# mochell/PiCLES

Hardware: AMD Instinct MI355X
Metric: particle_steps_per_sec (higher is better)
Workload: dtype f64

## Files before the change

### picles_amd/csrc/k_step.inc

```
#ifndef K_STEP_NAME
#define K_STEP_NAME k_step
#define K_STEP_WROW false
#include "k_step.inc"
#undef K_STEP_NAME
#undef K_STEP_WROW
#define K_STEP_NAME k_step_waverow
#define K_STEP_WROW true
#include "k_step.inc"
#undef K_STEP_NAME
#undef K_STEP_WROW
#else
template <bool FAST, bool TSIT, bool STATIC, bool METRIC, bool AUTO>
__global__ void __launch_bounds__(256, (FAST && !AUTO) ? 4 : (FAST ? 3 : 2)) K_STEP_NAME(KParams P, GridP G, Arrays A, double t_prev, double DT_prev,
                                                double t_start, double DT, int r0, int n0, int r1, int n1)
{
    constexpr bool WROW = K_STEP_WROW;
    static_assert(!WROW || (FAST && !METRIC), "k_step_waverow: specialised physics, Cartesian");
#ifdef PICLES_PHASE_CLOCK
    const unsigned long long pc0_ = __builtin_readcyclecounter();
    unsigned long long pc1_ = pc0_, pc2_ = pc0_, pc3_ = pc0_;
#endif
#ifdef PICLES_WAVE_LOG
    const unsigned long long wl0_ = __builtin_amdgcn_s_memrealtime();
    unsigned long long wl1_ = 0;
#endif
    dp_device_init(TSIT ? 1 : 0);
    order_sign_init();
    const long long ord_counts = order_counts(A);
    const int ord_entry = order_entry(A);
    const int mr_early = pull_reach_early(A);
    pm_device_init();
    long long t = 0;
    const unsigned int lblock = ordered_block(A, ord_counts, ord_entry);
    WaveRow wr = {0, 0, 0};
    const unsigned int lane = threadIdx.x & 63u;
    bool active;
    if constexpr (WROW) { active = rows_index_waverow(G, r0, n0, lblock, wr); t = wr.t0 + lane; }
    else active = rows_index(G, r0, n0, r1, n1, t, lblock);
    StepStats S = {{0u, 0u, 0u, 0}, 0u, 0u, 0u, 0u, 0u, 0u, 0};
    int rtile = -1, ccode = -1;
    if (active) {
        int i, jl;
        if constexpr (WROW) { i = wr.i0 + (int)lane; jl = wr.jl; }
        else { i = (int)(t % G.Nx); jl = (int)(t / G.Nx); }
        double s0 = 0.0, s1 = 0.0, s2 = 0.0;
        if constexpr (WROW) rmap_clear_ahead_waverow(A, wr, lane);
        else rmap_clear_ahead(A, t);
        const Arrays Av = WROW ? arrays_at(A, wr.t0) : A;
        const long long tx = WROW ? (long long)lane : t;
        constexpr bool PREFETCH = AUTO;
        unsigned char pf_pre = 0;
        Wind w_pre = {0.0, 0.0, 0.0, 0.0, 0.0, 0.0};
        double qold_pre = 0.0, uP_pre = 0.0, vP_pre = 0.0;
        int asw_pre = 0;
        if constexpr (PREFETCH) {
            pf_pre = Av.pflags[tx];
            w_pre = load_wind(P, Av, tx);
            if constexpr (WROW) w_pre.xi = (unsigned int)t;
            qold_pre = Av.qold[tx];
            asw_pre = Av.asw[tx];
            if (!STATIC) { uP_pre = Av.uP[tx]; vP_pre = Av.vP[tx]; }
        }
        if constexpr (WROW) {
            int cls;
            const int Rl = pull_reach_local_waverow(G, A, wr, lane, pull_reach(G, A, jl, mr_early), cls);
            pull_waverow(G, A, wr, lane, Rl, cls, s0, s1, s2);
        }
        else pull_any(G, A, i, jl, pull_reach_local(G, A, i, jl, pull_reach(G, A, jl, mr_early)), s0, s1, s2);
#ifdef PICLES_PHASE_CLOCK
        __asm__ volatile("" : "+v"(s0), "+v"(s1), "+v"(s2));
        pc1_ = __builtin_readcyclecounter();
#endif
#ifdef PICLES_WAVE_LOG
        __asm__ volatile("" : "+v"(s0), "+v"(s1), "+v"(s2));
        wl1_ = __builtin_amdgcn_s_memrealtime();
#endif
        unsigned char pf = PREFETCH ? pf_pre : Av.pflags[tx];
        __shared__ int stash_[WROW ? 1 : 5][256];
        if (pf & PF_STEPPED) {
            Wind w = PREFETCH ? w_pre : load_wind(P, Av, tx);
            if constexpr (WROW) w.xi = (unsigned int)t;
            Vec5 z = {0.0, 0.0, 0.0, 0.0, 0.0};
            double qold = PREFETCH ? qold_pre : Av.qold[tx], dtn = -1.0;
            int br = remesh_regs_lazy(P, pf, s0, s1, s2, DT_prev, z, STATIC ? &Av.u0[tx] : (PREFETCH ? &uP_pre : &Av.uP[tx]),
                                      STATIC ? &Av.v0[tx] : (PREFETCH ? &vP_pre : &Av.vP[tx]));
            int on = (br <= 1);
            int asw = AUTO ? (PREFETCH ? asw_pre : Av.asw[tx]) : 0;
            if (br == 1) { qold = PI_LNQOLDINIT; asw = ASW_FRESH; S.reseeds = 1; }
            unsigned int rs = S.reseeds;
            S.reseeds = 0;
            const int tid_ = threadIdx.x;
            if constexpr (WROW) stash_[0][tid_] = (int)pf | ((int)rs << 8);
            else {
                stash_[0][tid_] = (int)(unsigned int)((unsigned long long)t & 0xffffffffull); stash_[1][tid_] = (int)((unsigned long long)t >> 32);
                stash_[2][tid_] = i; stash_[3][tid_] = jl; stash_[4][tid_] = (int)pf | ((int)rs << 8);
            }
            int status;
            if (METRIC) status = advance_core<FAST, STATIC, true, TSIT, AUTO>(P, w, z, on, qold, dtn, t_start, DT, S, Av.m11[tx], Av.m22[tx], Av.pc[tx], &asw);
            else status = advance_core<FAST, STATIC, false, TSIT, AUTO>(P, w, z, on, qold, dtn, t_start, DT, S, 0.0, 0.0, 0.0, &asw);
#ifdef PICLES_PHASE_CLOCK
            __asm__ volatile("" : "+v"(z.lne));
            pc2_ = __builtin_readcyclecounter();
#endif
            KStepArgsPtr K = kargs_reload();
            const KParams Pb = K->P;
            const GridP Gb = K->G;
            const Arrays Ab = K->A;
            __asm__ volatile("" ::: "memory");
            const int tid2_ = threadIdx.x;
            WaveRow wrb = {0, 0, 0};
            long long tb;
            int ib = 0, jlb = 0, pr_;
            if constexpr (WROW) {
                wrb = waverow_of(Gb, K->r0, lblock);
                tb = wrb.t0 + (threadIdx.x & 63u);
                pr_ = stash_[0][tid2_];
            } else {
                tb = (long long)(((unsigned long long)(unsigned int)stash_[1][tid2_] << 32) | (unsigned int)stash_[0][tid2_]);
                ib = stash_[2][tid2_]; jlb = stash_[3][tid2_]; pr_ = stash_[4][tid2_];
            }
            const unsigned char pfb = (unsigned char)(pr_ & 0xff);
            const Arrays Abv = WROW ? arrays_at(Ab, wrb.t0) : Ab;
            const long long tbx = WROW ? (long long)(threadIdx.x & 63u) : tb;
            status = advance_guards(Pb, [&]() { Wind wg = load_wind(Pb, Abv, tbx); if constexpr (WROW) wg.xi = (unsigned int)tb; return wg; },
                                    z, dtn, K->t_start, K->DT, status, S);
            if (AUTO) Abv.asw[tbx] = asw;
            S.reseeds += (unsigned int)(pr_ >> 8);
            Abv.qold[tbx] = qold;
            Abv.status[tbx] = status;
            if constexpr (WROW) write_record_at(Gb, rec_row_out(Ab, Gb, wrb.jl + Gb.R) + wrb.i0, threadIdx.x & 63u, pfb, on, z, S, &ccode);
            else write_record(Gb, Ab, ib, jlb, pfb, on, z, S);
            rtile = WROW ? (int)(wrb.t0 >> 6) : (int)(tb >> 6);
        }
    }
    {
        KStepArgsPtr K = kargs_reload();
        const Arrays Ab = K->A;
        flush_stats<WROW>(Ab, S, rtile, ccode);
        if (Ab.ord && order_wanted(Ab)) order_file(Ab, lblock, __ballot(S.adv != 0 || S.reseeds != 0) != 0);
#ifdef PICLES_WAVE_LOG
        if ((threadIdx.x & 63) == 0) {
            unsigned int hw_, xcc_;
            __asm__ volatile("s_getreg_b32 %0, hwreg(HW_REG_HW_ID)" : "=s"(hw_));
            __asm__ volatile("s_getreg_b32 %0, hwreg(HW_REG_XCC_ID)" : "=s"(xcc_));
            unsigned long long *wl_ = (unsigned long long *)Ab.movie + 4ull * ((unsigned long long)lblock * 4ull + (threadIdx.x >> 6));
            wl_[0] = wl0_; wl_[1] = wl1_; wl_[2] = __builtin_amdgcn_s_memrealtime();
            wl_[3] = (unsigned long long)hw_ | ((unsigned long long)xcc_ << 32) | ((unsigned long long)blockIdx.x << 40);
        }
#endif
#ifdef PICLES_PHASE_CLOCK
        pc3_ = __builtin_readcyclecounter();
        if ((threadIdx.x & 63) == 0) {
            DevCounters *c = Ab.cnt + ((blockIdx.x * 4u + (threadIdx.x >> 6)) & (NSLOTS - 1));
            if (pc1_ == pc0_) pc1_ = pc3_;
            if (pc2_ < pc1_) pc2_ = pc1_;
            atomicAdd(&c->pad_[0], pc1_ - pc0_); atomicAdd(&c->pad_[1], pc2_ - pc1_); atomicAdd(&c->pad_[2], pc3_ - pc2_); atomicAdd(&c->pad_[3], 1ull);
        }
#endif
    }
}
#endif
```

### picles_amd/csrc/kernels.h

```cpp
#ifndef PICLES_KERNELS_H
#define PICLES_KERNELS_H

#include <hip/hip_runtime.h>
#include <cstdint>
#include <type_traits>

#include "../../include/picles_hip.h"
#include "physics.h"

struct GridP {
    int Nx, Ny;
    int periodic_x, periodic_y;
    int tripolar;
    int j_begin, ny_loc;
    int R;
    int Rp;
    int single_slab;
    int ngroups;
};

#define NSLOTS 1024
struct DevCounters {
    unsigned long long rhs, acc, rej, reseeds, clamps, maxit, adv, overflow;
    unsigned long long nonfinite, wslots, pad_[4];
// ... 575 lines not shown
                int jw = jj; if (jw < 0) jw += G.Ny; else if (jw >= G.Ny) jw -= G.Ny;
                row = jw + RO;
            } else {
                row = jl + dj + RO;
            }
            if (!rowok) continue;
#pragma unroll 1
            for (int si = 0; si < W; si++) {
                int qi = si + shx; if (qi >= W) qi -= W;
                int di = qi - R;
                int ii = i + di;
                if (ii < 0 || ii >= Nx) {
                    if (!G.periodic_x) continue;
                    ii += (ii < 0) ? Nx : -Nx;
                }
                pull_candidate(rec, (unsigned int)row * rowlen + (unsigned int)ii, pl, di, dj, grp, true, s0, s1, s2);
            }
        }
    }
}

__device__ __forceinline__ int floor_mod(int a, int b) { int r = a % b; return (r < 0) ? r + b : r; }

__device__ __forceinline__ void pull_node_tripolar(const GridP &G, const Arrays &A, int i, int jl, int R,
                                                   double &s0, double &s1, double &s2)
{
    const int RO = G.R, Nx = G.Nx, Ny = G.Ny, j = jl + G.j_begin, W = 2 * R + 1;
    const double *__restrict__ rec = A.rec;
    const unsigned int pl = (unsigned int)Nx, rowlen = 6u * pl;
    const int cB = floor_mod(Nx - 2 - i, Nx);
    const bool narrow = (2 * W <= Nx);
    const int a0 = floor_mod(i - R, Nx), b0 = floor_mod(cB - R, Nx);
    for (int grp = 1; grp <= G.ngroups; grp++) {
        for (int js = max(0, j - R); js < Ny; js++) {
            const unsigned int rbase = (unsigned int)(js - G.j_begin + RO) * rowlen;
            int ka = 0, kb = 0, is_full = 0;
            while (narrow ? (ka < W || kb < W) : (is_full < Nx)) {
                int is;
                if (narrow) {
                    const int wa = a0 + W - Nx, wb = b0 + W - Nx;
                    int ea = (ka < W) ? ((wa > 0) ? ((ka < wa) ? ka : a0 + (ka - wa)) : a0 + ka) : 0x7fffffff;
                    int eb = (kb < W) ? ((wb > 0) ? ((kb < wb) ? kb : b0 + (kb - wb)) : b0 + kb) : 0x7fffffff;
                    is = min(ea, eb);
                    if (ea == is) ka++;
                    if (eb == is) kb++;
                } else {
                    is = is_full++;
                }
                const int ci0 = (int)rec[rbase + 5u * pl + (unsigned int)is];
                if (ci0 == 0 || (ci0 & 3) != grp) continue;
                const int bx = ((ci0 >> 2) & 4095) - REC_BIAS, by = (ci0 >> 14) - REC_BIAS;
                const double wxh = rec[rbase + 3u * pl + (unsigned int)is], wyh = rec[rbase + 4u * pl + (unsigned int)is];
#pragma unroll
                for (int k = 0; k < 4; k++) {
                    const int ax = k & 1, ay = k >> 1;
                    int ci = is + bx + ax, cj = js + by + ay;
                    if (cj < 0) continue;
                    if (cj >= Ny) { ci = Nx - 1 - floor_mod(ci + 1, Nx); cj = 2 * Ny - 1 - cj; }
                    else ci = floor_mod(ci, Nx);
                    if (ci != i || cj != j) continue;
                    const double w = (ax ? wxh : 1.0 - wxh) * (ay ? wyh : 1.0 - wyh);
                    s0 += w * rec[rbase + (unsigned int)is];
                    s1 += w * rec[rbase + pl + (unsigned int)is];
                    s2 += w * rec[rbase + 2u * pl + (unsigned int)is];
                }
            }
        }
    }
}

__device__ __forceinline__ void pull_any(const GridP &G, const Arrays &A, int i, int jl, int R,
                                         double &s0, double &s1, double &s2)
{
    const int W = 2 * R + 1;
    if (R == 0) return;
    if (G.tripolar && jl + G.j_begin >= G.Ny - R) pull_node_tripolar(G, A, i, jl, R, s0, s1, s2);
    else if ((G.periodic_x && W > G.Nx) || (G.periodic_y && W > G.Ny)) pull_node_aliased(G, A, i, jl, R, s0, s1, s2);
    else if (R == 1) pull_node<1>(G, A, i, jl, 1, s0, s1, s2);
    else if (R == 2) pull_node<2>(G, A, i, jl, 2, s0, s1, s2);
    else if (R == 3) pull_node<3>(G, A, i, jl, 3, s0, s1, s2);
    else if (R == 4) pull_node<4>(G, A, i, jl, 4, s0, s1, s2);
    else pull_node<0>(G, A, i, jl, R, s0, s1, s2);
}

__device__ __forceinline__ int pull_reach_early(const Arrays &A) { return reach_counters(A)[A.mr_idx & 15]; }
__device__ __forceinline__ int pull_reach(const GridP &G, const Arrays &A, int jl, int m)
{
    if (G.Rp > 0 && (jl < G.R || jl >= G.ny_loc - G.R)) return G.Rp;
    if (m < 1) m = 1;
    return (G.Rp > 0 && m > G.Rp) ? G.Rp : m;
}
__device__ __forceinline__ int pull_reach(const GridP &G, const Arrays &A, int jl) { return pull_reach(G, A, jl, pull_reach_early(A)); }


__device__ __forceinline__ void rmap_clear_ahead(const Arrays &A, long long t)
{
    if ((t & 63) == 0) A.rmap[(size_t)((A.mr_idx >> 8) & 15) * (size_t)A.ntile + (size_t)(t >> 6)] = 0;
}


__device__ __forceinline__ int pull_reach_local(const GridP &G, const Arrays &A, int i, int jl, int Rg)
{
    int R = Rg;
    const int j = jl + G.j_begin;
    const bool edge_row = G.Rp > 0 && (jl < G.R || jl >= G.ny_loc - G.R);
    if (Rg >= 2 && Rg <= 31 && !edge_row && i - Rg >= 0 && i + Rg < G.Nx && jl - Rg >= 0 && jl + Rg < G.ny_loc &&
        j - Rg >= 0 && j + Rg < G.Ny) {
        const int *const rm = A.rmap + (size_t)(A.mr_idx & 15) * (size_t)A.ntile;
        int m = 0;
        long long t0 = (long long)(jl - Rg) * G.Nx + (i - Rg);
        for (int dj = -Rg; dj <= Rg; dj++, t0 += G.Nx) {
            const int a = rm[t0 >> 6], b = rm[(t0 + 2 * Rg) >> 6];
            m = max(m, max(a, b));
        }
        R = min(m, Rg);
    }
    if (Rg < 2) return Rg;
    int m = 0;
    while (__ballot(R > m)) m++;
    return m;
}

struct WaveRow {
    int jl, i0;
    long long t0;
};
__device__ __forceinline__ WaveRow waverow_of(const GridP &G, int r0, unsigned int lblock)
{
    const unsigned int nbx = (unsigned int)G.Nx >> 6;
    const unsigned int by = lblock / nbx, bx = lblock - by * nbx;
    WaveRow w;
    unsigned int tid = threadIdx.x;
    __asm__ volatile("" : "+v"(tid));
    w.jl = r0 + 4 * (int)by + __builtin_amdgcn_readfirstlane((int)(tid >> 6));
    w.i0 = (int)(64u * bx);
    w.t0 = (long long)w.jl * G.Nx + w.i0;
    return w;
}
__device__ __forceinline__ bool rows_index_waverow(const GridP &G, int r0, int n0, unsigned int lblock, WaveRow &w)
{
    const unsigned int nbx = (unsigned int)G.Nx >> 6;
    if (lblock / nbx >= ((unsigned int)n0 >> 2)) return false;
    w = waverow_of(G, r0, lblock);
    return true;
}
__device__ __forceinline__ Arrays arrays_at(const Arrays &A, long long t0)
{
    Arrays B = A;
    B.qold += t0; B.asw += t0; B.pflags += t0; B.status += t0;
    B.u0 += t0; B.v0 += t0; B.u1 += t0; B.v1 += t0; B.uP += t0; B.vP += t0;
    B.um = A.um ? A.um + t0 : nullptr; B.vm += t0;
    return B;
}
__device__ __forceinline__ void rmap_clear_ahead_waverow(const Arrays &A, const WaveRow &w, unsigned int lane)
{
    if (lane == 0u) {
        A.rmap[(size_t)((A.mr_idx >> 8) & 15) * (size_t)A.ntile + (size_t)(w.t0 >> 6)] = 0;
        class_map(A, (A.mr_idx >> 8) & 15)[(size_t)(w.t0 >> 6)] = 0;
    }
}

__device__ __forceinline__ int pull_reach_local_waverow(const GridP &G, const Arrays &A, const WaveRow &w, unsigned int lane, int Rg, int &cls)
{
    cls = 0;
    const bool klass = (A.mr_idx & MR_CLASS_ON) != 0;
    if (Rg < 2 && !klass) return Rg;
    const int jl = w.jl, j = jl + G.j_begin;
    const bool edge_row = G.Rp > 0 && (jl < G.R || jl >= G.ny_loc - G.R);
    if (Rg >= 1 && Rg <= 31 && !edge_row && w.i0 - Rg >= 0 && w.i0 + 63 + Rg < G.Nx && jl - Rg >= 0 && jl + Rg < G.ny_loc && j - Rg >= 0 && j + Rg < G.Ny) {
        const int *const rm = A.rmap + (size_t)(A.mr_idx & 15) * (size_t)A.ntile;
        const int *const cm = class_map(A, A.mr_idx & 15);
        const long long nbx = G.Nx >> 6;
        long long tile = ((long long)(jl - Rg) * G.Nx + w.i0) >> 6;
        int m = 0, diff = 0;
        const int c0 = klass ? cm[tile] : 0;
        for (int dj = -Rg; dj <= Rg; dj++, tile += nbx) {
            if (Rg >= 2) m = max(m, max(rm[tile - 1], max(rm[tile], rm[tile + 1])));
            if (klass) diff |= (cm[tile - 1] ^ c0) | (cm[tile] ^ c0) | (cm[tile + 1] ^ c0);
        }
        if (diff == 0 && c0 > 0) {
            int grp, bx, by;
            rec_decode((double)c0, grp, bx, by);
            const int rx = (bx < 0) ? -bx : bx + 1, ry = (by < 0) ? -by : by + 1;
            if (max(rx, ry) > Rg) diff = 1;
        }
        cls = __builtin_amdgcn_readfirstlane(diff == 0 ? c0 : 0);
        return Rg >= 2 ? __builtin_amdgcn_readfirstlane(min(m, Rg)) : Rg;
    }
    if (Rg < 2) return Rg;
    return pull_reach_local(G, A, w.i0 + (int)lane, jl, Rg);
}

template <int R>
__device__ __forceinline__ void pull_walk_lanes(const double *__restrict__ rec, unsigned int base, unsigned int pl, unsigned int rowlen,
                                                unsigned int m, unsigned int ax, unsigned int ay, double &s0, double &s1, double &s2)
{
    constexpr int W = 2 * R + 1;
    while (__ballot(m != 0u)) {
        double e[4], mx[4], my[4], wx[4], wy[4];
        bool on[4], hx[4], hy[4];
#pragma unroll
        for (int k = 0; k < 4; k++) {
            on[k] = (m != 0u);
            const int c = on[k] ? __builtin_ctz(m) : 0;
            m &= m - 1u;
            hx[k] = (ax >> c) & 1u; hy[k] = (ay >> c) & 1u;
            const unsigned int off = base + (unsigned int)((c / W - R) * (int)rowlen + (c % W - R));
            e[k] = mx[k] = my[k] = wx[k] = wy[k] = 0.0;
            if (on[k]) {
                wx[k] = rec[off + 3u * pl]; wy[k] = rec[off + 4u * pl];
                e[k] = rec[off]; mx[k] = rec[off + pl]; my[k] = rec[off + 2u * pl];
            }
        }
#pragma unroll
        for (int k = 0; k < 4; k++) {
            if (on[k]) {
                const double w = (hx[k] ? wx[k] : 1.0 - wx[k]) * (hy[k] ? wy[k] : 1.0 - wy[k]);
                s0 += w * e[k];
                s1 += w * mx[k];
                s2 += w * my[k];
            }
        }
    }
}

template <int R>
__device__ __forceinline__ void pull_window_waverow(const double *__restrict__ rec, const double *__restrict__ rec0, unsigned int lane,
                                                    unsigned int base, unsigned int pl, unsigned int rowlen, int grp,
                                                    double &s0, double &s1, double &s2)
{
    constexpr int W = 2 * R + 1, NC = W * W;
    static_assert(NC <= 25, "corner bits of all candidates in two words");
    const double *const codes = rec0 + 5u * (size_t)pl;
    unsigned int vo[5];
#pragma unroll
    for (int k = 0; k < 5; k++) vo[k] = 8u * ((unsigned int)k * pl + lane);
    int d[NC];
    unsigned int m0 = 0u, some = 0u, px = 0u, py = 0u;
#pragma unroll
    for (int c = 0; c < NC; c++) {
        const int di = c % W - R, dj = c / W - R;
        d[c] = (int)(codes + ((long long)dj * (long long)rowlen + di))[lane] - (grp + 4 * (REC_BIAS - 1 - di) + 4 * 4096 * (REC_BIAS - 1 - dj));
        const unsigned int n = (unsigned int)__builtin_popcountll(__ballot((d[c] & ~(4 | 16384)) == 0));
        m0 |= (n >> 6) << c;
        some |= n & 63u;
        px |= ((unsigned int)d[c] & 4u) << c;
        py |= (((unsigned int)d[c] >> 14) & 1u) << c;
    }
    if constexpr (R >= 2) {
        if (some != 0u) { pull_window_2p<R>(rec, base, pl, rowlen, grp, s0, s1, s2); return; }
    } else if (some != 0u) {
        unsigned int m = 0u, ax = 0u, ay = 0u;
#pragma unroll
        for (int c = 0; c < NC; c++) {
            m |= ((d[c] & ~(4 | 16384)) == 0 ? 1u : 0u) << c;
            ax |= ((d[c] & 4) ? 0u : 1u) << c;
            ay |= ((d[c] & 16384) ? 0u : 1u) << c;
        }
        pull_walk_lanes<R>(rec, base, pl, rowlen, m, ax, ay, s0, s1, s2);
        return;
    }
    unsigned int mu = m0;
    while (mu != 0u) {
        double e[4], mx[4], my[4], wx[4], wy[4];
        bool on[4], hx[4], hy[4];
#pragma unroll
        for (int k = 0; k < 4; k++) {
            on[k] = (mu != 0u);
            const int c = on[k] ? __builtin_ctz(mu) : 0;
            mu &= mu - 1u;
            hx[k] = !((px >> (c + 2)) & 1u); hy[k] = !((py >> c) & 1u);
            const double *const p = rec0 + ((long long)(c / W - R) * (long long)rowlen + (c % W - R));
            e[k] = mx[k] = my[k] = wx[k] = wy[k] = 0.0;
            if (on[k]) {
                const char *const pb = (const char *)p;
                wx[k] = *(const double *)(pb + vo[3]); wy[k] = *(const double *)(pb + vo[4]);
                e[k] = *(const double *)(pb + vo[0]); mx[k] = *(const double *)(pb + vo[1]); my[k] = *(const double *)(pb + vo[2]);
            }
        }
#pragma unroll
        for (int k = 0; k < 4; k++) {
            if (on[k]) {
                const double w = (hx[k] ? wx[k] : 1.0 - wx[k]) * (hy[k] ? wy[k] : 1.0 - wy[k]);
                s0 += w * e[k];
                s1 += w * mx[k];
                s2 += w * my[k];
            }
        }
    }
}

__device__ __forceinline__ void pull_class_waverow(const double *__restrict__ rec0, unsigned int lane, unsigned int pl, unsigned int rowlen,
                                                   int bx, int by, double &s0, double &s1, double &s2)
{
    unsigned int vo[5];
#pragma unroll
    for (int k = 0; k < 5; k++) vo[k] = 8u * ((unsigned int)k * pl + lane);
    double e[4], mx[4], my[4], wx[4], wy[4];
#pragma unroll
    for (int k = 0; k < 4; k++) {
        const int di = -bx - 1 + (k & 1), dj = -by - 1 + (k >> 1);
        const char *const pb = (const char *)(rec0 + ((long long)dj * (long long)rowlen + di));
        wx[k] = *(const double *)(pb + vo[3]); wy[k] = *(const double *)(pb + vo[4]);
        e[k] = *(const double *)(pb + vo[0]); mx[k] = *(const double *)(pb + vo[1]); my[k] = *(const double *)(pb + vo[2]);
    }
#pragma unroll
    for (int k = 0; k < 4; k++) {
        const bool hx = !(k & 1), hy = !(k >> 1);
        const double w = (hx ? wx[k] : 1.0 - wx[k]) * (hy ? wy[k] : 1.0 - wy[k]);
        s0 += w * e[k];
        s1 += w * mx[k];
        s2 += w * my[k];
    }
}

__device__ __forceinline__ void pull_waverow(const GridP &G, const Arrays &A, const WaveRow &w, unsigned int lane, int R, int cls,
                                             double &s0, double &s1, double &s2)
{
    const int j = w.jl + G.j_begin;
    if (cls != 0) {
        if (lane == 0u) {
            DevCounters *const c = A.cnt + ((blockIdx.x * 4u + (threadIdx.x >> 6)) & (NSLOTS - 1));
            atomicAdd(&c->cls, 1ull);
            if (cls == CMAP_EMPTY) atomicAdd(&c->cls_empty, 1ull);
        }
        if (cls == CMAP_EMPTY) return;
        int cgrp, bx, by;
        rec_decode((double)cls, cgrp, bx, by);
        const unsigned int pl = (unsigned int)G.Nx, rowlen = 6u * pl;
        const double *const rec0 = A.rec + ((size_t)(w.jl + G.R) * (size_t)rowlen + (size_t)w.i0);
        for (int grp = 1; grp <= G.ngroups; grp++)
// ... 34 lines not shown
```

### picles_amd/csrc/picles_hip.hip

```cpp
#include <hip/hip_runtime.h>
#include <hipcub/hipcub.hpp>

#include <algorithm>
#include <cstdint>
#include <cstdlib>
#include <cstdio>
#include <cstring>
#include <cmath>
#include <mutex>
#include <string>
#include <vector>

#include "../../include/picles_hip.h"
#include "physics.h"

#define PX_EXPORT extern "C" __attribute__((visibility("default")))

#include "kernels.h"
#include "k_diag.h"
#include "k_probe.h"
#include "k_stat.h"

__global__ void __launch_bounds__(256) k_seed(KParams P, GridP G, Arrays A, const signed char *mask, double seed_T)
{
// ... 1159 lines not shown
    hipLaunchKernelGGL(k_seed, dim3(nblocks(c->A.n, 256)), dim3(256), 0, c->stream, c->P, c->G, arrays_for(c, 0, 0), c->d_mask, c->od.timestep);
    HIPCHK(c, hipGetLastError());
    c->state_zero = false;
    c->seeded = true;
    return 0;
}

PX_EXPORT int32_t picles_zero_state(picles_ctx *c)
{
    if (!c) return -1;
    HIPCHK(c, hipSetDevice(c->device));
    { int rc = flush(c); if (rc) return rc; }
    if (c->ext_streams) HIPCHK(c, hipDeviceSynchronize());
    HIPCHK(c, hipMemsetAsync(c->A.state, 0, 3 * c->A.n * 8, c->stream));
    c->state_zero = true;
    return 0;
}

PX_EXPORT int32_t picles_tick(picles_ctx *c, double dt)
{
    if (!c) return -1;
    c->clock += dt;
    return 0;
}

PX_EXPORT int32_t picles_begin_step(picles_ctx *c, double dt, int32_t flags)
{
    if (!c) return -1;
    if (!(dt > 0.0)) return fail(c, -2, "dt must be positive");
    { int rc = flush(c); if (rc) return rc; }
    if (c->wind_grid_on) {
        HIPCHK(c, hipSetDevice(c->device));
        if (c->ext_streams && !c->ring_orders) HIPCHK(c, hipDeviceSynchronize());
        int rc = wind_grid_prepare(c, c->clock, dt, c->stream);
        if (rc) return rc;
    }
    c->step_dt = dt;
    c->step_flags = flags;
    c->edge_pending = false;
    c->cur ^= 1;
    c->mr_w = (c->mr_w + 1) % 5;
    if (c->cmap_hot > 0) c->cmap_hot--;
    return 0;
}

static bool physics_fast(const KParams &P) { return P.fast_phys != 0; }

static bool rows_of(const GridP &G, int which, int &r0, int &n0, int &r1, int &n1)
{
    int R = G.R;
    r0 = n0 = r1 = n1 = 0;
    bool small = G.ny_loc <= 2 * R;
    if (which == PICLES_ROWS_ALL) { n0 = G.ny_loc; }
    else if (which == PICLES_ROWS_EDGE) {
        if (small) n0 = G.ny_loc;
        else { n0 = R; r1 = G.ny_loc - R; n1 = R; }
    } else if (which == PICLES_ROWS_INTERIOR) {
        if (!small) { r0 = R; n0 = G.ny_loc - 2 * R; }
    } else return false;
    return true;
}
static int select_rows(picles_ctx *c, int which, int &r0, int &n0, int &r1, int &n1)
{
    return rows_of(c->G, which, r0, n0, r1, n1) ? 0 : fail(c, -2, "bad row selector");
}

static int step_prologue(picles_ctx *c, hipStream_t s)
{
    if (s != c->stream && !stream_idle(c->stream)) {
        HIPCHK(c, hipEventRecord(c->ev_ctx, c->stream));
        HIPCHK(c, hipStreamWaitEvent(s, c->ev_ctx, 0));
    }
    return 0;
}

PX_EXPORT int32_t picles_advance_rows(picles_ctx *c, int32_t which, void *stream)
{
    if (!c) return -1;
    HIPCHK(c, hipSetDevice(c->device));
    hipStream_t s = stream ? (hipStream_t)stream : c->stream;
    if (stream) c->ext_streams = true;
    int r0, n0, r1, n1;
    int rc = select_rows(c, which, r0, n0, r1, n1);
    if (rc) return rc;
    long long nt = (long long)(n0 + n1) * c->G.Nx;
    if (nt == 0) return 0;
    if ((rc = step_prologue(c, s))) return rc;
    c->ord_valid = false;
    if (c->cmap_hot > 0 && (rc = class_map_clear_rows(c, s, r0, n0, r1, n1))) return rc;
    timing_begin(c, s, 0);
    {
        const KParams &P = c->P;
        bool fast = physics_fast(P);
        if (!P.wind_static && P.wind_nk > 1) fast = false;
        Arrays A = arrays_for(c, c->cur, c->cur);
        StepLaunch L = {dim3(nblocks(nt, 256)), dim3(256), s, &c->P, &c->G, &A, 0.0, 0.0, c->clock, c->step_dt, r0, n0, r1, n1};
        launch_k_advance(L, fast, P.solver, P.wind_static != 0, c->A.pc != nullptr);
    }
    timing_end(c, s);
    HIPCHK(c, hipGetLastError());
    if (which == PICLES_ROWS_EDGE && s != c->stream) {
        HIPCHK(c, hipEventRecord(c->ev_edge, s));
        c->edge_pending = true;
    }
    return 0;
}

static bool step_fusable(const picles_ctx *c, int flags, double dt)
{
    if (flags != PICLES_STEP_ZERO_FIRST) return false;
    const KParams &P = c->P;
    if (c->wind_grid_on ? (c->wind_grid_mode != PICLES_LATTICE_SMOOTH3 && picles_lattice_knot_times(c->wg_t0, c->wg_dt, c->clock, dt, nullptr, 0) >= 2)
                        : (!P.wind_static && P.wind_nk > 1)) return false;
    const bool fast = physics_fast(P);
    if (c->wind_grid_on) return fast;
    if (c->A.pc) return fast && P.wind_static != 0;
    if (P.solver == 2) return fast && P.wind_static != 0;
    return P.wind_static != 0;
}

static bool step_rows_waverow(const picles_ctx *c, int which)
{
    int r0, n0, r1, n1;
    if (!rows_of(c->G, which, r0, n0, r1, n1)) return false;
    if (n0 + n1 == 0) return true;
    return waverow_flavour(physics_fast(c->P), c->A.pc != nullptr) && waverow_geometry(c->G.Nx, n0, n1);
}

static bool waverow_measured(const KParams &P) { return P.solver == 0 && P.wind_static != 0; }

static int launch_step_rows(picles_ctx *c, int which, hipStream_t s)
{
    int r0, n0, r1, n1;
    int rc = select_rows(c, which, r0, n0, r1, n1);
    if (rc) return rc;
    long long nt = (long long)(n0 + n1) * c->G.Nx;
    if (nt == 0) return 0;
    if ((rc = step_prologue(c, s))) return rc;
    const KParams &P = c->P;
    Arrays A = arrays_for(c, c->cur ^ 1, c->cur);
    bool fast = physics_fast(P);
    const bool orders = c->A.ord && (c->G.single_slab ? which == PICLES_ROWS_ALL : which == PICLES_ROWS_INTERIOR);
    if (orders) {
        A.nblk = (int)nblocks(nt, 256);
        const bool follows = c->ord_valid && c->ord_nblk == A.nblk;
        if (!follows) HIPCHK(c, hipMemsetAsync(c->A.ord, 0, (size_t)5 * (2 + c->A.nblk) * sizeof(int), s));
        A.ord_on = follows ? 1 : 0;
        c->ord_valid = true;
        c->ord_nblk = A.nblk;
    } else {
        A.ord = nullptr;
        if (c->G.single_slab || which != PICLES_ROWS_EDGE) c->ord_valid = false;
    }
    const bool waverow = (c->waverow_mode == 2 || (c->waverow_mode == 1 && waverow_measured(P))) && step_rows_waverow(c, which);
    if (waverow && c->pull_class) c->cmap_hot = 4;
    else if (!waverow && c->cmap_hot > 0 && (rc = class_map_clear_rows(c, s, r0, n0, r1, n1))) return rc;
    timing_begin(c, s, 0);
    {
        StepLaunch L = {dim3(nblocks(nt, 256)), dim3(256), s, &c->P, &c->G, &A, c->pend_t, c->pend_dt, c->clock, c->step_dt, r0, n0, r1, n1, waverow};
        if (fast && P.solver == 2) launch_k_step_auto(L, P.wind_static != 0, c->A.pc != nullptr);
        else launch_k_step_explicit(L, fast, P.solver, P.wind_static != 0, c->A.pc != nullptr);
    }
    timing_end(c, s);
    HIPCHK(c, hipGetLastError());
    return 0;
}

PX_EXPORT int32_t picles_begin_fused_step(picles_ctx *c, double dt)
{
    if (!c) return -1;
    if (!(dt > 0.0)) return fail(c, -2, "dt must be positive");
    if (!step_fusable(c, PICLES_STEP_ZERO_FIRST, dt)) return 1;
    if (c->waverow_mode == 2 && !(c->G.single_slab ? step_rows_waverow(c, PICLES_ROWS_ALL)
                                                   : step_rows_waverow(c, PICLES_ROWS_EDGE) && step_rows_waverow(c, PICLES_ROWS_INTERIOR)))
        return fail(c, -5, "PICLES_WAVEROW=require: a fused launch of this step does not qualify for k_step_waverow (one row range, "
                           "Nx a multiple of 64, rows a multiple of 4, specialised physics without the per-node metric)");
    HIPCHK(c, hipSetDevice(c->device));
    if (c->wind_grid_on) {
        Arrays &A = c->A;
        if (c->pending && !(c->wind_t1_valid && c->wind_t1 == c->clock && c->P.tw0 == c->pend_t && !c->P.wind_static))
            return 1;
        if (c->ext_streams && !c->ring_orders) HIPCHK(c, hipDeviceSynchronize());
        if (c->pending) {
            WindowPlan W;
            { int rc = wind_window_plan(c, c->clock, dt, W); if (rc) return rc; }
            if (!A.uP) {
                HIPCHK(c, hipMalloc(&A.uP, (size_t)A.n * 8));
                HIPCHK(c, hipMalloc(&A.vP, (size_t)A.n * 8));
            }
            double *tu = A.uP, *tv = A.vP;
            A.uP = A.u0; A.vP = A.v0;
            A.u0 = A.u1; A.v0 = A.v1;
            A.u1 = tu; A.v1 = tv;
            int rc = wind_window_sample(c, W, c->clock, dt, false, c->stream);
            if (rc) return rc;
        } else {
            int rc = wind_grid_prepare(c, c->clock, dt, c->stream);
            if (rc) return rc;
        }
        if (c->ext_streams && !c->ring_orders) HIPCHK(c, hipStreamSynchronize(c->stream));
    }
    c->step_dt = dt;
    c->step_flags = PICLES_STEP_ZERO_FIRST;
    c->edge_pending = false;
    c->cur ^= 1;
    c->mr_w = (c->mr_w + 1) % 5;
    if (c->cmap_hot > 0) c->cmap_hot--;
    return 0;
}

PX_EXPORT int32_t picles_step_rows(picles_ctx *c, int32_t which, void *stream)
{
    if (!c) return -1;
    HIPCHK(c, hipSetDevice(c->device));
    hipStream_t s = stream ? (hipStream_t)stream : c->stream;
    if (stream) c->ext_streams = true;
    if (!c->pending) return picles_advance_rows(c, which, stream);
    return launch_step_rows(c, which, s);
}

PX_EXPORT int32_t picles_end_fused_step(picles_ctx *c)
{
    if (!c) return -1;
    c->pending = true;
    c->pend_t = c->clock;
    c->pend_dt = c->step_dt;
    c->state_zero = false;
    c->edge_pending = false;
    step_completed(c);
    return 0;
}

static int launch_scatter(picles_ctx *c, hipStream_t s, bool remesh)
{
    Arrays A = arrays_for(c, c->cur, c->cur);
    int flags = c->step_flags;
    bool movie = (flags & PICLES_STEP_MOVIE) != 0;
    bool zero_first = (flags & PICLES_STEP_ZERO_FIRST) != 0;
    int accum = (zero_first || c->state_zero) ? 0 : 1;
    if (flags & PICLES_STEP_ATOMIC) {
        if (!c->G.single_slab) return fail(c, -5, "PICLES_STEP_ATOMIC is single-slab only");
        if (c->G.tripolar) return fail(c, -5, "PICLES_STEP_ATOMIC does not implement the tripolar fold: use the deterministic pull");
        if (!accum) HIPCHK(c, hipMemsetAsync(c->A.state, 0, 3 * c->A.n * 8, s));
        int ntx = (c->G.Nx + PT_TX - 1) / PT_TX, nty = (c->G.ny_loc + PT_TY - 1) / PT_TY;
        timing_begin(c, s, 1);
        hipLaunchKernelGGL(k_push_tiles<true>, dim3(ntx * nty), dim3(256), 0, s, c->G, A, ntx,
                           (const int *)nullptr, (const int *)nullptr, (const int *)nullptr,
                           (const double *)nullptr, (const double *)nullptr, 0LL);
        timing_end(c, s);
        HIPCHK(c, hipGetLastError());
        if (movie) HIPCHK(c, hipMemcpyAsync(c->A.movie, c->A.state, 3 * c->A.n * 8, hipMemcpyDeviceToDevice, s));
        if (remesh) {
            timing_begin(c, s, 2);
            hipLaunchKernelGGL(k_remesh, dim3(nblocks(c->A.n, 256)), dim3(256), 0, s, c->P, c->G, A, c->clock, c->step_dt);
            timing_end(c, s);
            HIPCHK(c, hipGetLastError());
        }
        if (movie && remesh) HIPCHK(c, hipMemsetAsync(c->A.state, 0, 3 * c->A.n * 8, s));
        c->state_zero = movie && remesh;
        return 0;
    }
    timing_begin(c, s, 1);
    if (remesh)
        hipLaunchKernelGGL(k_scatter<true>, dim3(nblocks(c->A.n, 256)), dim3(256), 0, s, c->P, c->G, A, accum, movie ? 1 : 0, c->clock, c->step_dt);
    else
        hipLaunchKernelGGL(k_scatter<false>, dim3(nblocks(c->A.n, 256)), dim3(256), 0, s, c->P, c->G, A, accum, 0, c->clock, c->step_dt);
    timing_end(c, s);
    HIPCHK(c, hipGetLastError());
    c->state_zero = movie && remesh;
    return 0;
}

PX_EXPORT int32_t picles_scatter_remesh(picles_ctx *c, void *stream)
{
    if (!c) return -1;
    HIPCHK(c, hipSetDevice(c->device));
    hipStream_t s = stream ? (hipStream_t)stream : c->stream;
    if (c->edge_pending) { HIPCHK(c, hipStreamWaitEvent(s, c->ev_edge, 0)); c->edge_pending = false; }
    int rc = step_prologue(c, s);
    if (rc || (rc = launch_scatter(c, s, true))) return rc;
    step_completed(c);
    return 0;
}

static int time_step_phases(picles_ctx *c, double dt, int32_t flags)
{
    if (step_fusable(c, flags, dt)) {
        int rc0 = picles_begin_fused_step(c, dt);
        if (rc0) return rc0 < 0 ? rc0 : fail(c, -6, "internal: fusable step refused");
        if ((rc0 = picles_step_rows(c, PICLES_ROWS_ALL, nullptr))) return rc0;
        return picles_end_fused_step(c);
    }
    int rc = picles_begin_step(c, dt, flags);
    if (rc) return rc;
    rc = picles_advance_rows(c, PICLES_ROWS_ALL, nullptr);
    if (rc) return rc;
    return picles_scatter_remesh(c, nullptr);
}

PX_EXPORT int32_t picles_time_step(picles_ctx *c, double dt, int32_t flags)
{
    if (!c) return -1;
    if (!c->G.single_slab) return fail(c, -5, "picles_time_step needs the whole grid; slabs use begin_step/advance_rows/scatter_remesh");
    if (!(dt > 0.0)) return fail(c, -2, "dt must be positive");
    { int rc = probe_room(c, 1, "picles_time_step"); if (rc) return rc; }
    int rc = time_step_phases(c, dt, flags);
    if (rc) return rc;
// ... 1372 lines not shown
```

Baseline: 8.181 billion.

## Stage u0/v0/qold into LDS via async global_load_lds in waverow static kernel

```diff
diff --git a/picles_amd/csrc/k_step.inc b/picles_amd/csrc/k_step.inc
--- a/picles_amd/csrc/k_step.inc
+++ b/picles_amd/csrc/k_step.inc
@@ -49,7 +49,12 @@
         const Arrays Av = WROW ? arrays_at(A, wr.t0) : A;
         const long long tx = WROW ? (long long)lane : t;
         constexpr bool PREFETCH = AUTO;
+        constexpr bool STAGE = WROW && STATIC && !AUTO;
         unsigned char pf_pre = 0;
+        if constexpr (STAGE) {
+            stage_fetch_waverow(Av, lane);
+            pf_pre = Av.pflags[tx];
+        }
         Wind w_pre = {0.0, 0.0, 0.0, 0.0, 0.0, 0.0};
         double qold_pre = 0.0, uP_pre = 0.0, vP_pre = 0.0;
         int asw_pre = 0;
@@ -75,13 +80,14 @@
         __asm__ volatile("" : "+v"(s0), "+v"(s1), "+v"(s2));
         wl1_ = __builtin_amdgcn_s_memrealtime();
 #endif
-        unsigned char pf = PREFETCH ? pf_pre : Av.pflags[tx];
+        unsigned char pf = (PREFETCH || STAGE) ? pf_pre : Av.pflags[tx];
         __shared__ int stash_[WROW ? 1 : 5][256];
         if (pf & PF_STEPPED) {
-            Wind w = PREFETCH ? w_pre : load_wind(P, Av, tx);
+            if constexpr (STAGE) stage_wait_waverow();
+            Wind w = PREFETCH ? w_pre : (STAGE ? stage_wind_waverow(lane) : load_wind(P, Av, tx));
             if constexpr (WROW) w.xi = (unsigned int)t;
             Vec5 z = {0.0, 0.0, 0.0, 0.0, 0.0};
-            double qold = PREFETCH ? qold_pre : Av.qold[tx], dtn = -1.0;
+            double qold = PREFETCH ? qold_pre : (STAGE ? (*stage_of_wave())[STAGE_QOLD][lane] : Av.qold[tx]), dtn = -1.0;
             int br = remesh_regs_lazy(P, pf, s0, s1, s2, DT_prev, z, STATIC ? &Av.u0[tx] : (PREFETCH ? &uP_pre : &Av.uP[tx]),
                                       STATIC ? &Av.v0[tx] : (PREFETCH ? &vP_pre : &Av.vP[tx]));
             int on = (br <= 1);
diff --git a/picles_amd/csrc/kernels.h b/picles_amd/csrc/kernels.h
--- a/picles_amd/csrc/kernels.h
+++ b/picles_amd/csrc/kernels.h
@@ -751,11 +751,76 @@
     B.um = A.um ? A.um + t0 : nullptr; B.vm += t0;
     return B;
 }
+#define STAGE_U0 0
+#define STAGE_V0 1
+#define STAGE_QOLD 2
+typedef double StagePlanes[3][64];
+__device__ __forceinline__ StagePlanes *stage_of_wave()
+{
+    __shared__ __attribute__((aligned(16))) double stage_[4][3][64];
+    unsigned int tid = threadIdx.x;
+    __asm__ volatile("" : "+v"(tid));
+    return &stage_[__builtin_amdgcn_readfirstlane((int)(tid >> 6))];
+}
+__device__ __forceinline__ void stage_fetch_waverow(const Arrays &Av, unsigned int lane)
+{
+    typedef __attribute__((address_space(3))) void *lds_ptr;
+    StagePlanes &st = *stage_of_wave();
+    if (lane < 32u) {
+        __builtin_amdgcn_global_load_lds(Av.u0 + 2u * lane, (lds_ptr)&st[STAGE_U0][0], 16, 0, 0);
+        __builtin_amdgcn_global_load_lds(Av.v0 + 2u * lane, (lds_ptr)&st[STAGE_V0][0], 16, 0, 0);
+        __builtin_amdgcn_global_load_lds(Av.qold + 2u * lane, (lds_ptr)&st[STAGE_QOLD][0], 16, 0, 0);
+    }
+}
+__device__ __forceinline__ void stage_wait_waverow()
+{
+    __builtin_amdgcn_s_waitcnt(0x0f70);
+    __asm__ volatile("" ::: "memory");
+}
+__device__ __forceinline__ Wind stage_wind_waverow(unsigned int lane)
+{
+    const StagePlanes &st = *stage_of_wave();
+    Wind w;
+    w.u0 = st[STAGE_U0][lane]; w.v0 = st[STAGE_V0][lane];
+    w.du = 0.0; w.dv = 0.0; w.bu = 0.0; w.bv = 0.0;
+    w.xi = 0u;
+    return w;
+}
+static inline bool stage_aligned(const Arrays &A) { return (((uintptr_t)A.u0 | (uintptr_t)A.v0 | (uintptr_t)A.qold) & 15u) == 0; }
+
 __device__ __forceinline__ void rmap_clear_ahead_waverow(const Arrays &A, const WaveRow &w, unsigned int lane)
 {
     if (lane == 0u) {
         A.rmap[(size_t)((A.mr_idx >> 8) & 15) * (size_t)A.ntile + (size_t)(w.t0 >> 6)] = 0;
         class_map(A, (A.mr_idx >> 8) & 15)[(size_t)(w.t0 >> 6)] = 0;
+    }
+}
+
+template <int R>
+__device__ __forceinline__ void map_rows_waverow(const int *rm, const int *cm, long long tile, long long nbx, bool klass, int &m, int &diff, int &c0)
+{
+    constexpr int W = 2 * R + 1;
+    int c[W][3];
+    c0 = 0;
+    if (klass) {
+#pragma unroll
+        for (int k = 0; k < W; k++)
+#pragma unroll
+            for (int q = 0; q < 3; q++) c[k][q] = cm[tile + k * nbx + (q - 1)];
+    }
+    if (R >= 2) {
+        int r[W][3];
+#pragma unroll
+        for (int k = 0; k < W; k++)
+#pragma unroll
+            for (int q = 0; q < 3; q++) r[k][q] = rm[tile + k * nbx + (q - 1)];
+#pragma unroll
+        for (int k = 0; k < W; k++) m = max(m, max(r[k][0], max(r[k][1], r[k][2])));
+    }
+    if (klass) {
+        c0 = c[0][1];
+#pragma unroll
+        for (int k = 0; k < W; k++) diff |= (c[k][0] ^ c0) | (c[k][1] ^ c0) | (c[k][2] ^ c0);
     }
 }
 
@@ -772,10 +837,15 @@
         const long long nbx = G.Nx >> 6;
         long long tile = ((long long)(jl - Rg) * G.Nx + w.i0) >> 6;
         int m = 0, diff = 0;
-        const int c0 = klass ? cm[tile] : 0;
-        for (int dj = -Rg; dj <= Rg; dj++, tile += nbx) {
-            if (Rg >= 2) m = max(m, max(rm[tile - 1], max(rm[tile], rm[tile + 1])));
-            if (klass) diff |= (cm[tile - 1] ^ c0) | (cm[tile] ^ c0) | (cm[tile + 1] ^ c0);
+        int c0;
+        if (Rg == 1) map_rows_waverow<1>(rm, cm, tile, nbx, klass, m, diff, c0);
+        else if (Rg == 2) map_rows_waverow<2>(rm, cm, tile, nbx, klass, m, diff, c0);
+        else {
+            c0 = klass ? cm[tile] : 0;
+            for (int dj = -Rg; dj <= Rg; dj++, tile += nbx) {
+                m = max(m, max(rm[tile - 1], max(rm[tile], rm[tile + 1])));
+                if (klass) diff |= (cm[tile - 1] ^ c0) | (cm[tile] ^ c0) | (cm[tile + 1] ^ c0);
+            }
         }
         if (diff == 0 && c0 > 0) {
             int grp, bx, by;
diff --git a/picles_amd/csrc/picles_hip.hip b/picles_amd/csrc/picles_hip.hip
--- a/picles_amd/csrc/picles_hip.hip
+++ b/picles_amd/csrc/picles_hip.hip
@@ -1335,7 +1335,9 @@
         A.ord = nullptr;
         if (c->G.single_slab || which != PICLES_ROWS_EDGE) c->ord_valid = false;
     }
-    const bool waverow = (c->waverow_mode == 2 || (c->waverow_mode == 1 && waverow_measured(P))) && step_rows_waverow(c, which);
+    const bool staged = P.wind_static != 0 && !(fast && P.solver == 2);
+    const bool waverow = (c->waverow_mode == 2 || (c->waverow_mode == 1 && waverow_measured(P))) && step_rows_waverow(c, which) &&
+                         (!staged || stage_aligned(A));
     if (waverow && c->pull_class) c->cmap_hot = 4;
     else if (!waverow && c->cmap_hot > 0 && (rc = class_map_clear_rows(c, s, r0, n0, r1, n1))) return rc;
     timing_begin(c, s, 0);
```

Result: faster. 8.322 billion, median of 6 (+1.7%).
